# zhangzhousuper/Radish_PT

Measured on AMD Instinct MI355X. Metric: Mrays/s, higher is better.
Workload: dtype f32

## Files before the change

include/radish_hip.h:

```cpp
#ifndef RADISH_HIP_H
#define RADISH_HIP_H
#include <stdint.h>

#ifdef __cplusplus
extern "C" {
#endif

#define RDH_OK 0
#define RDH_ERR_ARGS (-1)
#define RDH_ERR_NO_SCENE (-2)
#define RDH_ERR_UNSUPPORTED (-3)
#define RDH_ERR_NO_DEVICE (-4)
#define RDH_ERR_STATE (-5)
#define RDH_ERR_COMM (-6)

typedef struct rdh_ctx rdh_ctx;

typedef struct rdh_texture { int32_t width, height; const float *data; } rdh_texture;

typedef struct rdh_scene_desc {
    const float *vertices;
    const float *normals;
    const float *texcoords;
    const float *boundingBoxes;
// ... 35 lines not shown
    uint64_t anyRays;
    uint64_t nodeVisits;
    uint64_t triTests;
    uint64_t closestHits;
} rdh_counters;

#define RDH_PT_MEGAKERNEL 0u
#define RDH_PT_WAVEFRONT 1u
#define RDH_PT_SORT_MATERIAL 2u
#define RDH_PT_COUNT 4u
#define RDH_PT_PERSISTENT 16u
#define RDH_PT_ONE_LANE_PER_PIXEL 64u
#define RDH_PT_MEGA_GBUFFER RDH_PT_ONE_LANE_PER_PIXEL
#define RDH_PT_WG_PER_RAY 256u
#define RDH_PT_NO_DEFER 128u
#define RDH_PT_PARTITION_GBUFFER 512u
#define RDH_PT_WF_SUBFRAMES 2048u
#define RDH_PT_RESTIR_FUSED 1024u
#define RDH_PT_WF_SMALL_LISTS 4096u
#define RDH_PT_PAIRS 32768u
#define RDH_PT_NO_PAIRS 16384u
#define RDH_PT_NO_PACKETS 8192u
#define RDH_PT_AUTO 65536u
#define RDH_PT_NO_SCHEDULE 32u
#define RDH_PT_PROFILE 8u

#define RDH_REUSE_TEMPORAL 1
#define RDH_REUSE_SPATIAL 2

typedef struct rdh_restir_params {
    int32_t reuseMask;
    int32_t risCount;
    int32_t numSpatial;
    int32_t temporalClamp;
    int32_t faithfulRIS;
} rdh_restir_params;

int rdh_create(rdh_ctx **out, int device);
void rdh_destroy(rdh_ctx *ctx);
const char *rdh_last_error(const rdh_ctx *ctx);
int rdh_set_stream(rdh_ctx *ctx, void *hipStream);
int rdh_synchronize(rdh_ctx *ctx);

int rdh_scene_upload(rdh_ctx *ctx, const rdh_scene_desc *desc);
typedef struct rdh_light_update {
    const void *lightSampler;
// ... 90 lines not shown
                                    const float *d_momentAccumIn, const float *d_colorIn, const rdh_gbuffer *gb, int first);
int rdh_denoise_estimate_variance(rdh_ctx *ctx, float *d_variance, const float *d_moment, int width, int height);
int rdh_denoise_filter_variance(rdh_ctx *ctx, float *d_varianceOut, const float *d_varianceIn, int width, int height);

int rdh_restir_read(rdh_ctx *ctx, int which, void *hostOut);
long long rdh_restir_read_scratch(rdh_ctx *ctx, int which, void *hostOut, long long maxBytes);

int rdh_trace_closest(rdh_ctx *ctx, const float *d_rays, int64_t n, rdh_hit *d_hits, uint32_t flags);
int rdh_trace_occluded(rdh_ctx *ctx, const float *d_segments, int64_t n, int32_t *d_occluded, uint32_t flags);

int rdh_dump_rays(rdh_ctx *ctx, int looper, int maxDepth, float *d_closest, int64_t capClosest, float *d_any, int64_t capAny,
                  int64_t *nClosest, int64_t *nAny);
int rdh_set_occupancy_share(rdh_ctx *ctx, int share);

int rdh_counters_reset(rdh_ctx *ctx);
int rdh_counters_read(rdh_ctx *ctx, rdh_counters *out);

int rdh_profile_reset(rdh_ctx *ctx);
int rdh_profile_read(rdh_ctx *ctx, double *totalMs, int64_t *launches);

int rdh_debug_persist_stamps(rdh_ctx *ctx, uint64_t *out5x4096);
int rdh_debug_persist_phases(rdh_ctx *ctx, uint64_t *out16);
int rdh_debug_wf_stamps(rdh_ctx *ctx, uint64_t *out, int64_t capacity, int32_t *stages, int32_t *waves);

int rdh_last_kernel_ms(rdh_ctx *ctx, float *ms);

#ifdef __cplusplus
}
#endif
#endif
```

radish_pt_amd/_build.py:

```python
import os
import subprocess
import sys

ROOT = os.path.dirname(os.path.dirname(os.path.abspath(__file__)))
CSRC = os.path.join(ROOT, "radish_pt_amd", "csrc")
HIPCC = os.environ.get("HIPCC", "/opt/rocm/bin/hipcc")

HOST_SOURCES = [os.path.join(CSRC, "host", "scene_build.cpp"), os.path.join(CSRC, "host", "scene_load.cpp")]
HIP_SOURCES = [os.path.join(CSRC, "radish_hip.hip")]
HIP_DEPS = [
    os.path.join(CSRC, "device", f)
    for f in ("rmath.h", "layouts.h", "traverse.h", "bsdf.h", "lights.h", "path_step.h", "kernels_pt.h", "kernels_restir.h", "kernels_wave.h", "kernels_persist.h", "kernels_walk.h", "wg_trace.h", "kernels_display.h", "kernels_denoise.h", "kernels_bvh.h", "kernels_refit.h", "kernels_lbvh.h", "kernels_lights.h", "kernels_pose.h", "kernels_materials.h", "kernels_textures.h", "display_math.h", "denoise_math.h", "reservoir.h")
] + [os.path.join(ROOT, "include", "radish_hip.h")]

HIP_FLAGS = [
    "--offload-arch=gfx950", "-O3", "-std=c++17", "-fPIC", "-shared", "-ffp-contract=off", "-fno-fast-math",
    "-fno-gpu-rdc", "-Wall", "-Wno-unused-function", "-Wno-unused-value", "-Wno-unused-result",
]


def _newer(target, deps):
    if not os.path.exists(target):
        return True
    t = os.path.getmtime(target)
    return any(os.path.exists(d) and os.path.getmtime(d) > t for d in deps)


def _run(cmd):
    print("[build]", " ".join(cmd), flush=True)
    subprocess.check_call(cmd)


def build_host(force=False):
    out = os.path.join(CSRC, "libradish_host.so")
    deps = HOST_SOURCES + [os.path.join(ROOT, "include", "radish_host.h")]
# ... 76 lines not shown
```

radish_pt_amd/api.py:

```python
import ctypes as C
import os

import numpy as np

from . import hostlib
from . import layouts as L

_HERE = os.path.dirname(os.path.abspath(__file__))
HIP_LIB_PATH = os.environ.get("RADISH_HIP_LIB") or os.path.join(_HERE, "csrc", "libradish_hip.so")

RDH_PT_MEGAKERNEL, RDH_PT_WAVEFRONT, RDH_PT_SORT_MATERIAL, RDH_PT_COUNT, RDH_PT_PROFILE = 0, 1, 2, 4, 8
RDH_PT_PERSISTENT = 16
RDH_PT_NO_SCHEDULE = 32
RDH_PT_ONE_LANE_PER_PIXEL = 64
RDH_PT_MEGA_GBUFFER = RDH_PT_ONE_LANE_PER_PIXEL
RDH_PT_NO_DEFER = 128
RDH_PT_WG_PER_RAY = 256
RDH_PT_PARTITION_GBUFFER = 512
RDH_PT_RESTIR_FUSED = 1024
RDH_PT_WF_SUBFRAMES = 2048
RDH_PT_WF_SMALL_LISTS = 4096
RDH_PT_NO_PAIRS = 16384
RDH_PT_NO_PACKETS = 8192
RDH_PT_PAIRS = 32768
RDH_PT_AUTO = 65536
RDH_BVH_SAH, RDH_BVH_LBVH = 0, 1
BVH_BUILDERS = {"sah": RDH_BVH_SAH, "lbvh": RDH_BVH_LBVH}
RDH_POSE_REFIT, RDH_POSE_SAH, RDH_POSE_LBVH = 0, 1, 2
RDH_POSE_REBUILD_LIGHTS = 1
POSE_TREES = {"refit": RDH_POSE_REFIT, "sah": RDH_POSE_SAH, "lbvh": RDH_POSE_LBVH}
OBJECT_RANGE_DTYPE = np.dtype([("firstPrim", "<i4"), ("numPrims", "<i4"), ("restFirstPrim", "<i4")])
SOBOL_SAMPLE_NUM = 10000

EXPORTS = [
    "rdh_create", "rdh_destroy", "rdh_last_error", "rdh_set_stream", "rdh_synchronize", "rdh_scene_upload",
    "rdh_scene_free", "rdh_set_camera", "rdh_set_partition", "rdh_tiles_per_rank", "rdh_untile", "rdh_path_trace", "rdh_path_trace_samples",
    "rdh_path_trace_direct", "rdh_gbuffer_render", "rdh_restir_init", "rdh_restir_free", "rdh_restir_direct",
    "rdh_restir_read", "rdh_restir_read_scratch", "rdh_copy_image_to_pbo", "rdh_denoise_eaw", "rdh_denoise_svgf", "rdh_denoise_modulate",
    "rdh_denoise_add", "rdh_denoise_temporal_accumulate", "rdh_denoise_estimate_variance", "rdh_denoise_filter_variance", "rdh_restir_exchange_pack", "rdh_restir_exchange_unpack", "rdh_trace_closest", "rdh_trace_occluded", "rdh_counters_reset", "rdh_counters_read",
    "rdh_last_kernel_ms", "rdh_profile_reset", "rdh_profile_read", "rdh_debug_persist_stamps", "rdh_debug_persist_phases", "rdh_debug_wf_stamps",
    "rdh_gbuffer_exchange_pack", "rdh_gbuffer_exchange_unpack", "rdh_comm_unique_id", "rdh_comm_init", "rdh_comm_destroy",
    "rdh_dump_rays", "rdh_set_occupancy_share", "rdh_allgather_tiles", "rdh_path_trace_gathered", "rdh_restir_exchange", "rdh_restir_direct_gathered", "rdh_gbuffer_exchange",
    "rdh_comm_init_all", "rdh_path_trace_gathered_all", "rdh_gbuffer_exchange_all", "rdh_restir_direct_gathered_all",
    "rdh_comm_set_overlap", "rdh_comm_join",
    "rdh_build_bvh_device", "rdh_scene_update_geometry", "rdh_debug_read_tree",
    "rdh_scene_refit_geometry", "rdh_scene_tree_cost",
    "rdh_build_bvh_device_ex", "rdh_scene_update_geometry_ex",
    "rdh_scene_track_motion",
    "rdh_build_alias_table_device", "rdh_scene_rebuild_lights", "rdh_debug_read_lights",
    "rdh_scene_set_objects", "rdh_scene_pose_objects", "rdh_debug_read_world",
    "rdh_scene_set_materials", "rdh_build_light_list_device",
    "rdh_scene_set_texture", "rdh_scene_env_power", "rdh_debug_read_textures",
    "rdh_scene_set_geometry", "rdh_debug_read_geometry",
]


class SceneDescC(C.Structure):
    _fields_ = [
        ("vertices", C.c_void_p), ("normals", C.c_void_p), ("texcoords", C.c_void_p), ("boundingBoxes", C.c_void_p),
        ("bvhNodes", C.c_void_p * 6), ("bvhSize", C.c_int32), ("numPrims", C.c_int32),
        ("materialIds", C.c_void_p), ("materials", C.c_void_p), ("numMaterials", C.c_int32),
        ("numLights", C.c_int32), ("lightPrimIds", C.c_void_p), ("lightUnitRadiance", C.c_void_p),
        ("sumLightPowerInv", C.c_float), ("lightSamplerLength", C.c_int32), ("lightSampler", C.c_void_p),
# ... 723 lines not shown

    def profile_reset(self):
        self.check(lib().rdh_profile_reset(self.h))

    def profile_read(self):
        ms, n = C.c_double(0), C.c_int64(0)
        self.check(lib().rdh_profile_read(self.h, C.byref(ms), C.byref(n)))
        return ms.value, n.value

    def debug_persist_stamps(self):
        out = np.zeros((5, 4096), dtype=np.uint64)
        self.check(lib().rdh_debug_persist_stamps(self.h, out.ctypes.data))
        return out

    def debug_wf_stamps(self):
        fn = lib().rdh_debug_wf_stamps
        fn.argtypes, fn.restype = [C.c_void_p, C.c_void_p, C.c_int64, C.POINTER(C.c_int32), C.POINTER(C.c_int32)], C.c_int32
        stages, waves = C.c_int32(0), C.c_int32(0)
        self.check(fn(self.h, None, 0, C.byref(stages), C.byref(waves)))
        out = np.zeros((stages.value, waves.value, 6), dtype=np.uint64)
        self.check(fn(self.h, out.ctypes.data, out.size, C.byref(stages), C.byref(waves)))
        return out

    def debug_persist_phases(self):
        out = np.zeros(16, dtype=np.uint64)
        self.check(lib().rdh_debug_persist_phases(self.h, out.ctypes.data))
        return out

    def last_kernel_ms(self):
        ms = C.c_float(0)
        self.check(lib().rdh_last_kernel_ms(self.h, C.byref(ms)))
        return ms.value


class ReservoirReuse:
    NONE, Temporal, Spatial, TemporalSpatial = 0, 1, 2, 3


class Settings:
    traceDepth = 0
    useReservoir = True
    reservoirReuse = ReservoirReuse.Temporal
    accumulate = False
    ptFlags = RDH_PT_PERSISTENT
    restirNumSpatial = 5
    restirRISCount = 32
# ... 262 lines not shown
```

radish_pt_amd/csrc/device/kernels_wave.h:

```cpp
#pragma once
#include "kernels_pt.h"
#include "wg_trace.h"

namespace rd {

constexpr int kWfLitCap = 8192;
constexpr int kWfLitShadow = 0x40000000;
constexpr int kMaxWaveDepth = 32;

struct alignas(128) WaveCounter {
    int v;
    int pad[31];
};
#ifndef RD_WF_TICKET_SHARDS
#define RD_WF_TICKET_SHARDS 8
#endif
constexpr int kTicketShards = RD_WF_TICKET_SHARDS;
struct WaveCounters {
    WaveCounter rayCount[kMaxWaveDepth + 2];
    WaveCounter shadowCount[kMaxWaveDepth + 2];
    WaveCounter litCount[kMaxWaveDepth + 2];
    WaveCounter traceHead[kMaxWaveDepth + 2];
    WaveCounter shadeHead[kMaxWaveDepth + 2][4];
    WaveCounter traceTicket[kMaxWaveDepth + 2][kTicketShards];
    WaveCounter shadeTicket[kMaxWaveDepth + 2][kTicketShards];
};

struct WaveWorkspace {
    float4 *ro[2];
    float4 *rd[2];
    float4 *thr[2];
    float4 *prevPos[2];
    float4 *accD;
    float4 *accI;
    float4 *nee[2];
    float4 *sht[2];
    uint2 *rng[2];
    int4 *hit;
    int *rayq[2];
    int *shadowq;
    int *litq[2];
    int litCap;
    int *treeOvf;
    int treeOvfDepth;
// ... 11 lines not shown
    const unsigned tag = __float_as_uint(n.w), kind = tag & 3u;
    if (kind == kWfNeeNone) return;
    float4 *acc = (kind == 0u ? w.accD : w.accI) + (tag >> 2);
    const float4 a = *acc;
    *acc = make_float4(a.x + n.x, a.y + n.y, a.z + n.z, 0.f);
}

RD_DEV Ray wfSlotRay(const WaveWorkspace &w, int set, int p, bool shadow, float &limit) {
    if (shadow) {
        const float4 x = w.prevPos[set][p], y = w.sht[set][p];
        return shadowRay(mk3(x.x, x.y, x.z), mk3(y.x, y.y, y.z), limit);
    }
    const float4 o = w.ro[set][p], d = w.rd[set][p];
    limit = 3.402823466e+38f;
    return Ray{mk3(o.x, o.y, o.z), mk3(d.x, d.y, d.z)};
}

struct WaveSlotPath {
    const WaveWorkspace &w;
    const int rs, p;
    const int wr, q;
    int home;
    const bool delta;
    RD_DEV v3 throughput() {
        const float4 t = w.thr[rs][p];
        home = __float_as_int(t.w);
        return mk3(t.x, t.y, t.z);
    }
    RD_DEV float samplePdf() const { return w.ro[rs][p].w; }
    RD_DEV bool sampleDelta() const { return delta; }
    RD_DEV v3 prevPos() const { const float4 c = w.prevPos[rs][p]; return mk3(c.x, c.y, c.z); }
    RD_DEV void setDirect(v3 v) { w.accD[home] = make_float4(v.x, v.y, v.z, 0.f); }
    RD_DEV void addIndirect(v3 v) { const float4 a = w.accI[home]; w.accI[home] = make_float4(a.x + v.x, a.y + v.y, a.z + v.z, 0.f); }
    RD_DEV Sampler rng(const DScene &s) const { const uint2 r = w.rng[rs][p]; return Sampler{s.sobol, r.x, (int)r.y}; }
    RD_DEV void setNee(v3 c, float nw) { w.nee[wr][q] = make_float4(c.x, c.y, c.z, wfNeeTag(home, nw < 0.f ? kWfNeeNone : (nw == 0.f ? 0u : 1u))); }
    RD_DEV void setPrevPos(v3 x) { w.prevPos[wr][q] = make_float4(x.x, x.y, x.z, 0.f); }
    RD_DEV void setRay(const Ray &ray, float pdf, bool deltaSample, v3 throughput, const Sampler &rng) {
        w.ro[wr][q] = make_float4(ray.o.x, ray.o.y, ray.o.z, pdf);
        w.rd[wr][q] = make_float4(ray.d.x, ray.d.y, ray.d.z, deltaSample ? 1.f : 0.f);
        w.thr[wr][q] = make_float4(throughput.x, throughput.y, throughput.z, __int_as_float(home));
        w.rng[wr][q] = make_uint2(rng.scramble, (unsigned)rng.ptr);
    }
};


RD_DEV void waveAppend(bool pred, int item, int *queue, int *count) {
    unsigned long long mask = __ballot(pred);
    if (mask == 0ull) return;
    int leader = __ffsll((long long)mask) - 1;
    int base = 0;
    if ((int)(threadIdx.x & 63u) == leader) base = atomicAdd(count, __popcll(mask));
    base = __shfl(base, leader, 64);
    if (pred) queue[base + __popcll(mask & laneMaskLt())] = item;
}

constexpr int kShadeChunks = 4;
constexpr int kShadePacket = 64 * kShadeChunks;
RD_DEV void waveAppendN(const bool (&pred)[kShadeChunks], const int (&item)[kShadeChunks], int *queue, int *count) {
// ... 380 lines not shown
        const unsigned long long doneM = __ballot(!alive && p >= 0);
        if (doneM != 0ull && __popcll(doneM) * 64 >= (__popcll(doneM) + __popcll(__ballot(alive))) * RD_WF_FINISH_MIN)
        if (!alive && p >= 0) {
            if (isShadow) {
                if (!occluded) wfAddNee(w, w.nee[set][p]);
            } else {
                bool hit = hitPrim != -1;
                if (hit) nHits++;
                w.hit[p] = make_int4(hitPrim, __float_as_int(hit ? hitBary.x : 0.f), __float_as_int(hit ? hitBary.y : 0.f),
                                     hit ? int(s.primClass[hitPrim]) : 0);
            }
            p = -1;
        }
    }
    RD_WF_STAMP(2);
    if (COUNT) flushCounters(s.counters, nClosest, nAny, nHits, ws);
}

constexpr int kSortChunks = 16;
constexpr int kSortPacket = 64 * kSortChunks;
#ifndef RD_WF_SHADE_WAVES
#define RD_WF_SHADE_WAVES 1
#endif
__global__ __launch_bounds__(256, RD_WF_SHADE_WAVES) void k_wf_shade(DScene s, WaveWorkspace w, int k, int maxDepth, int sorted) {
    __shared__ int sSorted[4][kSortPacket];
    WaveCounters *c = w.ctr;
    const int wg = workgroupTicket(c->shadeTicket[k]);
    const int lane = int(threadIdx.x & 63u);
    int *mySorted = sSorted[threadIdx.x >> 6];
    {
        const int q = 0;
        const int n = c->rayCount[k].v;
        const int *hitq = w.rayq[k & 1];
        int pendP[kShadeChunks], pendQ[kShadeChunks];
        bool pendShadow[kShadeChunks], pendRay[kShadeChunks];
#pragma unroll
        for (int j = 0; j < kShadeChunks; j++) {
            pendP[j] = pendQ[j] = -1;
            pendShadow[j] = pendRay[j] = false;
        }
        int packet = kShadePacket;
        if (sorted) {
            const int perWave = n / (2 * gridWaves());
            packet = ((perWave + kShadePacket - 1) / kShadePacket) * kShadePacket;
            packet = packet < kShadePacket ? kShadePacket : (packet > kSortPacket ? kSortPacket : packet);
        }
        int packetEnd = 0;
        for (int base = logicalWave(wg) * packet, sub = 0, fresh = 1;;) {
            if (sub == packet) {
// ... 26 lines not shown
                        if (in) mySorted[at + __popcll(m & laneMaskLt())] = pp[j];
                        at += __popcll(m);
                    }
                }
                __builtin_amdgcn_wave_barrier();
            }
            int item = base + sub + lane;
            const int subNow = sub;
            sub += 64;
            bool active = sorted ? (subNow + lane < packetEnd) : (item < n);
            bool emitShadow = false, emitRay = false, litShadow = false, litRay = false, rayFirst = false;
            int p = -1;
            const int q = base + subNow + lane;
            if (active) {
                p = sorted ? mySorted[subNow + lane] : hitq[item];
                if (p <= -2) p = -2 - p;
                active = p >= 0;
            }
            if (active) {
                const int4 h = w.hit[p];
                const float4 rdw = w.rd[k & 1][p];
                WaveSlotPath st{w, k & 1, p, (k + 1) & 1, q, p, rdw.w != 0.f};
                const PathStepResult r = pathStep(s, k, maxDepth, h.x, mk2(__int_as_float(h.y), __int_as_float(h.z)), mk3(rdw.x, rdw.y, rdw.z), st);
                if (r.shadow) {
                    w.sht[(k + 1) & 1][q] = make_float4(r.shadowTo.x, r.shadowTo.y, r.shadowTo.z, 0.f);
                    emitShadow = true;
                    const v3 dl = r.shadowTo - r.shadowFrom;
                    const float l2 = dot(dl, dl) * 1.21e-12f;
                    litShadow = dl.x * dl.x < l2 || dl.y * dl.y < l2 || dl.z * dl.z < l2;
                }
                if (r.extension) {
                    emitRay = true;
                    litRay = fabs_(r.ray.d.x) < 1.1e-6f || fabs_(r.ray.d.y) < 1.1e-6f || fabs_(r.ray.d.z) < 1.1e-6f;
                }
            }
            if (__ballot(litShadow || litRay) != 0ull) {
                int *lq = w.litq[(k + 1) & 1];
                int *lc = &c->litCount[k + 1].v;
                for (int kind = 0; kind < 2; kind++) {
                    const bool pred = kind == 0 ? litShadow : litRay;
                    const unsigned long long m = __ballot(pred);
                    if (m == 0ull) continue;
                    int at = 0;
                    if (lane == 0) at = atomicAdd(lc, __popcll(m));
                    at = __shfl(at, 0, 64) + __popcll(m & laneMaskLt());
                    if (pred && at < w.litCap) {
                        lq[at] = kind == 0 ? (q | kWfLitShadow) : q;
                        if (kind == 0) emitShadow = false;
                        else rayFirst = true;
                    }
                }
            }
            {
                const int j = ((sub >> 6) - 1) & (kShadeChunks - 1);
#pragma unroll
                for (int jj = 0; jj < kShadeChunks; jj++)
                    if (jj == j) {
                        pendP[jj] = q;
                        pendQ[jj] = rayFirst ? -2 - q : q;
                        pendShadow[jj] = emitShadow;
                        pendRay[jj] = emitRay;
                    }
            }
            if ((sub & (kShadePacket - 1)) == 0 || base + sub >= n) {
                waveAppendN(pendShadow, pendP, w.shadowq, &c->shadowCount[k].v);
                waveAppendN(pendRay, pendQ, w.rayq[(k + 1) & 1], &c->rayCount[k + 1].v);
#pragma unroll
                for (int jj = 0; jj < kShadeChunks; jj++) pendShadow[jj] = pendRay[jj] = false;
// ... 30 lines not shown
```

radish_pt_amd/csrc/radish_hip.hip:

```cpp
#include "radish_hip.h"

#include <hip/hip_runtime.h>
#include <dlfcn.h>

#include <algorithm>
#include <cfloat>
#include <climits>
#include <cmath>
#include <cstdarg>
#include <cstdio>
#include <cstring>
#include <mutex>
#include <string>
#include <type_traits>
#include <utility>
#include <vector>

#include "device/kernels_pt.h"
#include "device/kernels_restir.h"
#include "device/kernels_wave.h"
#include "device/kernels_persist.h"
#include "device/kernels_walk.h"
#include "device/kernels_display.h"
#include "device/kernels_denoise.h"
// ... 55 lines not shown
        epoch = 0;
    }
    void beginCall() {
        if (++epoch == 0) {
            std::fill(stamp.begin(), stamp.end(), 0u);
            epoch = 1;
        }
    }
    bool marked(size_t id) const { return stamp[id] == epoch; }
    bool mark(size_t id) {
        if (marked(id)) return false;
        stamp[id] = epoch;
        return true;
    }
};

struct SceneState {
    bool haveScene = false;
    DScene ds{};
    std::vector<void *> sceneAllocs;

    int *dLightPrims = nullptr;
    int numLights = 0;
    PairRec *updPairs = nullptr;
    bool treePending = false;

    bool planValid = false;
    bool treeRefit = false;

    TriRec *prevTris = nullptr;
    bool movedSinceRender = false;

    void *lightScratch = nullptr;
    bool lightsPending = false;

    std::vector<rdh_object_range> objects;
    StampSet posed;
    PoseArgs pose{};
    bool worldStale = false;

    std::vector<HostMaterial> hostMats;
    std::vector<int> matPrims;
    StampSet edited;
    int numTextures = 0;
    int lightCap = 0;
    int lightLenCap = 0;
// ... 49 lines not shown
    float4 *restirState = nullptr;
    long long restirPixels = 0;
    GrowBuf splitBuf{bufs};
    long long splitLastSlots = 0;
    bool restirFirstFrame = true;

    std::vector<hipEvent_t> profEvents;
    size_t profUsed = 0;

    void *comm = nullptr;
    hipStream_t commStream = nullptr;
    hipEvent_t evToComm = nullptr, evGbuf = nullptr, evImg = nullptr, evResv = nullptr;
    bool commOverlap = true;
    bool gbufPending = false;
    bool resvPending = false;
    GrowBuf commSend[2] = {GrowBuf{bufs}, GrowBuf{bufs}}, commRecv{bufs};

    WaveWorkspace wf[kWfParts] = {};
    hipStream_t wfStream = nullptr;
    hipEvent_t evWfJoin3 = nullptr;
    long long wfCapacity = 0;
    std::vector<void *> wfAllocs;
    hipEvent_t evWfFork = nullptr, evWfJoin = nullptr;
#ifdef RD_WF_STAMPS
    GrowBuf wfStamps{bufs};
    int wfStampStages = 0, wfStampWaves = 0;
#endif

    GrowBuf bvhScratch{bufs};
    GrowBuf lbvhScratch{bufs};
    GrowBuf updTree{bufs};
    GrowBuf dTreeHdr{bufs};
    GrowBuf hTreeHdr{bufs, true};
    hipEvent_t evTree = nullptr;
    StagePair aliasStage{bufs};
    hipEvent_t evUpdWait = nullptr;

    GrowBuf refitBuf{bufs};

    GrowBuf aliasScratch{bufs};
    GrowBuf hLightSums{bufs, true};
    hipEvent_t evLights = nullptr;

    StagePair poseStage{bufs};
    GrowBuf dPoseStage{bufs};

// ... 458 lines not shown
                return rc;
        }
        if ((rc = wfAlloc(c, &w.accD, n)) || (rc = wfAlloc(c, &w.accI, n)) ||
            (rc = wfAlloc(c, &w.hit, n)) || (rc = wfAlloc(c, &w.rayq[0], n)) || (rc = wfAlloc(c, &w.rayq[1], n)) ||
            (rc = wfAlloc(c, &w.shadowq, n)) || (rc = wfAlloc(c, &w.ctr, 1)) || (rc = wfAlloc(c, &w.litq[0], (size_t)kWfLitCap)) ||
            (rc = wfAlloc(c, &w.litq[1], (size_t)kWfLitCap)))
            return rc;
        w.litCap = 0;
    }
    if (!c->evWfFork) {
        int rc;
        if ((rc = newEvent(c, &c->evWfFork)) || (rc = newEvent(c, &c->evWfJoin))) return rc;
        HIP_TRY(c, hipStreamCreateWithFlags(&c->wfStream, hipStreamNonBlocking));
        if ((rc = newEvent(c, &c->evWfJoin3))) return rc;
    }
    c->wfCapacity = slots;
    return RDH_OK;
}

int wavefrontPathTrace(rdh_ctx *c, const PixelMap &pm, float *d_direct, float *d_indirect, int iter, int looper, int samples,
                       int maxDepth, uint32_t flags) {
    if (maxDepth > kMaxWaveDepth) return fail(c, RDH_ERR_ARGS, "maxDepth %d exceeds %d", maxDepth, kMaxWaveDepth);
    const bool count = (flags & RDH_PT_COUNT) != 0, sort = (flags & RDH_PT_SORT_MATERIAL) != 0;
    const bool tree = usePairs(c, flags);
    unsigned traceRes = 0, shadeRes = 0;
    int rq = RDH_OK;
    withBools([&](auto cnt, auto pr) { rq = residentGrid(c, k_wf_trace<cnt.value, pr.value>, 256, &traceRes); }, count, tree);
    if (rq || (rq = residentGrid(c, k_wf_shade, 256, &shadeRes))) return rq;
    if (tree && !count) {
        int cus = 0;
        if (int rc = cuCount(c, &cus)) return rc;
        traceRes = std::min(traceRes, (unsigned)cus * (unsigned)RD_WF_PAIR_MAX_WAVES);
    }
    const unsigned traceGrid = sharedGrid(c, std::min(traceRes, kPersistentGrid), kUnbounded);
    const unsigned shadeGrid = sharedGrid(c, std::min(shadeRes, kPersistentGrid), kUnbounded);
    static const int partsEnv = getenv("RADISH_WF_PARTS") ? atoi(getenv("RADISH_WF_PARTS")) : kWfPartsDefault;
    int parts = ((flags & RDH_PT_WF_SUBFRAMES) && pm.numBlocks >= 2048) ? (partsEnv >= 1 && partsEnv <= kWfParts ? partsEnv : kWfPartsDefault) : 1;
    const int ovfDepth = c->scene.ds.treeDepth + 1;
    const size_t ovfNeed = (size_t)traceGrid * 4 * 64 * (size_t)ovfDepth * 2;
    if (tree && parts > 1 && (size_t)parts * ovfNeed * sizeof(int) > kWfStripBudget) parts = 1;
    hipStream_t sts[kWfParts] = {c->stream, c->sideStream, c->wfStream};
    if (tree) {
        for (int h = 0; h < parts; h++) {
            if (int rc = grow(c, c->wfTreeOvf[h], ovfNeed, ovfNeed * sizeof(int), Busy::Device)) return rc;
            c->wf[h].treeOvf = c->wfTreeOvf[h].as<int>();
            c->wf[h].treeOvfDepth = ovfDepth;
        }
    }
#ifdef RD_WF_STAMPS
    {
        const size_t stamps = (size_t)(maxDepth + 1) * traceGrid * 4 * kWfStampKinds + (size_t)(maxDepth + 1);
        if (int rc = grow(c, c->wfStamps, stamps, stamps * sizeof(unsigned long long), Busy::Device)) return rc;
        HIP_TRY(c, hipMemsetAsync(c->wfStamps.p, 0, stamps * sizeof(unsigned long long), c->stream));
        for (int h = 0; h < kWfParts; h++) {
            c->wf[h].stamps = h == 0 ? c->wfStamps.as<unsigned long long>() : nullptr;
            c->wf[h].stampWaves = (int)(traceGrid * 4);
            c->wf[h].stampStages = maxDepth + 1;
        }
        c->wfStampStages = maxDepth + 1;
        c->wfStampWaves = (int)(traceGrid * 4);
    }
#endif
    const long pf = parts >= 2 ? profBegin(c, flags) : -1;
    if (parts >= 2) {
        HIP_TRY(c, hipEventRecord(c->evWfFork, c->stream));
        for (int h = 1; h < parts; h++) HIP_TRY(c, hipStreamWaitEvent(sts[h], c->evWfFork, 0));
    }
    int rc = RDH_OK;
    auto keep = [&](hipError_t e, const char *what) {
        if (e != hipSuccess && rc == RDH_OK) rc = fail(c, (int)e, "HIP error (%s:%d): %s: %s", __FILE__, __LINE__, what, hipGetErrorString(e));
    };
    for (int h = 0; h < parts; h++) {
        const unsigned waves = traceGrid * 4u;
        c->wf[h].litCap = (int)(waves * 64u < (unsigned)kWfLitCap ? waves * 64u : (unsigned)kWfLitCap);
        if (flags & RDH_PT_WF_SMALL_LISTS) c->wf[h].litCap = 4;
    }
    for (int h = 0; h < parts; h++) {
        hipStream_t st = sts[h];
        WaveWorkspace &w = c->wf[h];
        const unsigned nLocal = (unsigned)(pm.numBlocks - h + parts - 1) / (unsigned)parts;
        const unsigned gridBlk = (((nLocal * (unsigned)samples + 3u) / 4u + 7u) / 8u) * 8u;
        keep(hipMemsetAsync(w.ctr, 0, sizeof(WaveCounters), st), "hipMemsetAsync(wavefront counters)");
        hipLaunchKernelGGL(k_wf_raygen, dim3(gridBlk), dim3(256), 0, st, c->scene.ds, c->cam, pm, w, looper, samples, h, parts);
    }
    for (int k = 0; k <= maxDepth && rc == RDH_OK; k++) {
        for (int h = 0; h < parts; h++) {
            hipStream_t st = sts[h];
            WaveWorkspace &w = c->wf[h];
            long pe = (h == 0 && parts == 1) ? profBegin(c, flags) : -1;
            withBools([&](auto cnt, auto pr) {
                hipLaunchKernelGGL((k_wf_trace<cnt.value, pr.value>), dim3(traceGrid), dim3(256), 0, st, c->scene.ds, w, k);
            }, count, tree);
            profEnd(c, pe);
            hipLaunchKernelGGL(k_wf_shade, dim3(shadeGrid), dim3(256), 0, st, c->scene.ds, w, k, maxDepth, sort ? 1 : 0);
        }
        keep(hipGetLastError(), "wavefront stage launch");
    }
    for (int h = 0; h < parts && rc == RDH_OK; h++) {
        hipStream_t st = sts[h];
        const unsigned nLocal = (unsigned)(pm.numBlocks - h + parts - 1) / (unsigned)parts;
        const unsigned gridBlk = (((nLocal + 3u) / 4u + 7u) / 8u) * 8u;
        hipLaunchKernelGGL(k_wf_finish, dim3(gridBlk), dim3(256), 0, st, pm, c->wf[h], iter, samples, d_direct, d_indirect, h, parts);
    }
    keep(hipGetLastError(), "k_wf_finish");
    if (parts >= 2) {
        hipError_t e1 = hipEventRecord(c->evWfJoin, c->sideStream);
        hipError_t e2 = hipStreamWaitEvent(c->stream, c->evWfJoin, 0);
        hipError_t e3 = hipEventRecord(c->evWfJoin3, c->wfStream);
        hipError_t e4 = hipStreamWaitEvent(c->stream, c->evWfJoin3, 0);
        if (e1 != hipSuccess || e2 != hipSuccess || e3 != hipSuccess || e4 != hipSuccess) {
            hipStreamSynchronize(c->sideStream);
            hipStreamSynchronize(c->wfStream);
            keep(e1 != hipSuccess ? e1 : (e2 != hipSuccess ? e2 : (e3 != hipSuccess ? e3 : e4)), "wavefront join");
        }
    }
    profEnd(c, pf);
    return rc;
// ... 327 lines not shown
                               const_cast<LightPre *>(c->scene.ds.lightPre), (int)lights.size(), d->sumLightPowerInv);
            HIP_TRY(c, hipStreamSynchronize(c->stream));
        }
    }
    std::vector<AliasRec> alias(d->lightSamplerLength);
    if (d->lightSamplerLength) memcpy(alias.data(), d->lightSampler, sizeof(AliasRec) * alias.size());
    for (auto &e : alias)
        if (e.failId < 0 || e.failId >= d->lightSamplerLength) return fail(c, RDH_ERR_ARGS, "alias table failId out of range");
    if ((rc = uploadVec(c, alias, &c->scene.ds.lightAlias))) return rc;
    std::vector<uint32_t> sobol(d->sampleSequence, d->sampleSequence + 10000 * 200);
    if ((rc = uploadVec(c, sobol, &c->scene.ds.sobol))) return rc;

    c->scene.ds.counters = c->dCounters;
    c->scene.ds.bvhSize = S;
    c->scene.ds.numPrims = N;
    c->scene.ds.lightSamplerLength = d->lightSamplerLength;
    c->scene.ds.sumLightPowerInv = d->sumLightPowerInv;
    c->scene.lightCap = d->numLights;
    c->scene.lightLenCap = d->lightSamplerLength;
    c->scene.primCap = N;
    c->scene.hostMats.assign(hm, hm + d->numMaterials);
    c->scene.matPrims.assign((size_t)d->numMaterials, 0);
    for (int p = 0; p < N; p++) c->scene.matPrims[(size_t)d->materialIds[p]]++;
    c->scene.edited.reset((size_t)d->numMaterials);
    c->scene.numTextures = d->numTextures;
    c->scene.texInfo.assign(texInfo.begin(), texInfo.begin() + d->numTextures);
    c->scene.texFloats = texFloats;
    c->scene.haveScene = true;
    c->orderValid = false;
    return RDH_OK;
}

int rdh_set_camera(rdh_ctx *c, const void *camera196) {
    if (!c || !camera196) return RDH_ERR_ARGS;
    DCamera d = toDeviceCamera(camera196);
    if (d.resx <= 0 || d.resy <= 0) return fail(c, RDH_ERR_ARGS, "camera resolution %dx%d", d.resx, d.resy);
    if (d.resx != c->cam.resx || d.resy != c->cam.resy) c->orderValid = false;
    c->cam = d;
    c->haveCamera = true;
    return RDH_OK;
}

int rdh_set_partition(rdh_ctx *c, int rank, int world, int tileSize) {
    if (!c || world < 1 || rank < 0 || rank >= world || tileSize < 8 || (tileSize % 8) != 0)
        return fail(c, RDH_ERR_ARGS, "rdh_set_partition(rank=%d, world=%d, tile=%d)", rank, world, tileSize);
    if (rank != c->rank || world != c->world || tileSize != c->tile) c->orderValid = false;
// ... 1027 lines not shown
#ifdef RD_PERSIST_STAMPS
    HIP_TRY(c, hipStreamSynchronize(c->stream));
    HIP_TRY(c, hipMemcpy(out5x4096, c->dPersist->stamp, sizeof(unsigned long long) * 5 * 4096, hipMemcpyDeviceToHost));
    return RDH_OK;
#else
    return fail(c, RDH_ERR_UNSUPPORTED, "library built without RD_PERSIST_STAMPS");
#endif
}

int rdh_debug_wf_stamps(rdh_ctx *c, uint64_t *out, int64_t capacity, int32_t *stages, int32_t *waves) {
    if (!c || !stages || !waves || capacity < 0 || (capacity > 0 && !out)) return RDH_ERR_ARGS;
#ifdef RD_WF_STAMPS
    HIP_TRY(c, hipStreamSynchronize(c->stream));
    *stages = c->wfStampStages;
    *waves = c->wfStampWaves;
    const int64_t n = (int64_t)c->wfStampStages * c->wfStampWaves * kWfStampKinds;
    if (n > 0 && capacity >= n) HIP_TRY(c, hipMemcpy(out, c->wfStamps.p, sizeof(unsigned long long) * (size_t)n, hipMemcpyDeviceToHost));
    return RDH_OK;
#else
    return fail(c, RDH_ERR_UNSUPPORTED, "library built without RD_WF_STAMPS");
#endif
}

int rdh_copy_image_to_pbo(rdh_ctx *c, void *d_pbo, const void *d_image, int width, int height, int kind, int toneMapping,
                          float scale) {
    if (!c) return RDH_ERR_ARGS;
    if (!d_pbo || !d_image || width <= 0 || height <= 0 || kind < 0 || kind > 3 || toneMapping < 0 || toneMapping > 2)
        return fail(c, RDH_ERR_ARGS, "rdh_copy_image_to_pbo: bad arguments");
    HIP_TRY(c, hipSetDevice(c->device));
    if (int rj = joinComm(c)) return rj;
    long long total = (long long)width * height;
    hipLaunchKernelGGL(k_send_image_to_pbo, dim3((unsigned)((total + 255) / 256)), dim3(256), 0, c->stream,
                       static_cast<uint32_t *>(d_pbo), d_image, width, height, kind, toneMapping, scale);
    HIP_TRY(c, hipGetLastError());
    return RDH_OK;
}

extern "C++" {
namespace {
int denoiseGB(rdh_ctx *c, const rdh_gbuffer *gb, DenoiseGB &d, const char *what) {
    if (int rj = joinComm(c)) return rj;
    if (!gb || !gb->albedo || !gb->motion || gb->frameIdx < 0 || gb->frameIdx > 1 || gb->width <= 0 || gb->height <= 0)
        return fail(c, RDH_ERR_ARGS, "%s: bad G-buffer", what);
    for (int k = 0; k < 2; k++)
        if (!gb->normal[k] || !gb->depth[k] || !gb->primId[k]) return fail(c, RDH_ERR_ARGS, "%s: null G-buffer plane", what);
    const int f = gb->frameIdx;
// ... 1280 lines not shown
```

Baseline: 3063.

## Cull last-bounce rays missing emitter bounds and skip zero-contribution shadow rays

In the wavefront shade kernel, extension rays at the final bounce are no longer emitted when they cannot hit the bounding box of all emissive triangles (only with no environment map and a complete light list). Shadow rays whose NEE contribution is zero or absent are also no longer queued. A small per-frame kernel computes the padded emitter box. This cuts trace work on the last stage and on useless shadow rays, at the cost of an extra tiny launch, an extra atomic per wave for lit-shadow counting, and a new debug counter API.

```diff
diff --git a/include/radish_hip.h b/include/radish_hip.h
--- a/include/radish_hip.h
+++ b/include/radish_hip.h
@@ -81,6 +81,7 @@
 #define RDH_PT_NO_PAIRS 16384u
 #define RDH_PT_NO_PACKETS 8192u
 #define RDH_PT_AUTO 65536u
+#define RDH_PT_WALK_ALL 131072u
 #define RDH_PT_NO_SCHEDULE 32u
 #define RDH_PT_PROFILE 8u
 
@@ -217,6 +218,7 @@
 int rdh_debug_persist_stamps(rdh_ctx *ctx, uint64_t *out5x4096);
 int rdh_debug_persist_phases(rdh_ctx *ctx, uint64_t *out16);
 int rdh_debug_wf_stamps(rdh_ctx *ctx, uint64_t *out, int64_t capacity, int32_t *stages, int32_t *waves);
+int rdh_debug_wf_counts(rdh_ctx *ctx, int32_t *rays, int32_t *shadows, int32_t capacity, int32_t *stages);
 
 int rdh_last_kernel_ms(rdh_ctx *ctx, float *ms);
 
diff --git a/radish_pt_amd/_build.py b/radish_pt_amd/_build.py
--- a/radish_pt_amd/_build.py
+++ b/radish_pt_amd/_build.py
@@ -10,7 +10,7 @@
 HIP_SOURCES = [os.path.join(CSRC, "radish_hip.hip")]
 HIP_DEPS = [
     os.path.join(CSRC, "device", f)
-    for f in ("rmath.h", "layouts.h", "traverse.h", "bsdf.h", "lights.h", "path_step.h", "kernels_pt.h", "kernels_restir.h", "kernels_wave.h", "kernels_persist.h", "kernels_walk.h", "wg_trace.h", "kernels_display.h", "kernels_denoise.h", "kernels_bvh.h", "kernels_refit.h", "kernels_lbvh.h", "kernels_lights.h", "kernels_pose.h", "kernels_materials.h", "kernels_textures.h", "display_math.h", "denoise_math.h", "reservoir.h")
+    for f in ("rmath.h", "layouts.h", "traverse.h", "bsdf.h", "lights.h", "path_step.h", "kernels_pt.h", "kernels_restir.h", "kernels_wave.h", "ray_cull.h", "kernels_persist.h", "kernels_walk.h", "wg_trace.h", "kernels_display.h", "kernels_denoise.h", "kernels_bvh.h", "kernels_refit.h", "kernels_lbvh.h", "kernels_lights.h", "kernels_pose.h", "kernels_materials.h", "kernels_textures.h", "display_math.h", "denoise_math.h", "reservoir.h")
 ] + [os.path.join(ROOT, "include", "radish_hip.h")]
 
 HIP_FLAGS = [
diff --git a/radish_pt_amd/api.py b/radish_pt_amd/api.py
--- a/radish_pt_amd/api.py
+++ b/radish_pt_amd/api.py
@@ -24,6 +24,7 @@
 RDH_PT_NO_PACKETS = 8192
 RDH_PT_PAIRS = 32768
 RDH_PT_AUTO = 65536
+RDH_PT_WALK_ALL = 131072
 RDH_BVH_SAH, RDH_BVH_LBVH = 0, 1
 BVH_BUILDERS = {"sah": RDH_BVH_SAH, "lbvh": RDH_BVH_LBVH}
 RDH_POSE_REFIT, RDH_POSE_SAH, RDH_POSE_LBVH = 0, 1, 2
@@ -39,6 +40,7 @@
     "rdh_restir_read", "rdh_restir_read_scratch", "rdh_copy_image_to_pbo", "rdh_denoise_eaw", "rdh_denoise_svgf", "rdh_denoise_modulate",
     "rdh_denoise_add", "rdh_denoise_temporal_accumulate", "rdh_denoise_estimate_variance", "rdh_denoise_filter_variance", "rdh_restir_exchange_pack", "rdh_restir_exchange_unpack", "rdh_trace_closest", "rdh_trace_occluded", "rdh_counters_reset", "rdh_counters_read",
     "rdh_last_kernel_ms", "rdh_profile_reset", "rdh_profile_read", "rdh_debug_persist_stamps", "rdh_debug_persist_phases", "rdh_debug_wf_stamps",
+    "rdh_debug_wf_counts",
     "rdh_gbuffer_exchange_pack", "rdh_gbuffer_exchange_unpack", "rdh_comm_unique_id", "rdh_comm_init", "rdh_comm_destroy",
     "rdh_dump_rays", "rdh_set_occupancy_share", "rdh_allgather_tiles", "rdh_path_trace_gathered", "rdh_restir_exchange", "rdh_restir_direct_gathered", "rdh_gbuffer_exchange",
     "rdh_comm_init_all", "rdh_path_trace_gathered_all", "rdh_gbuffer_exchange_all", "rdh_restir_direct_gathered_all",
@@ -808,6 +810,16 @@
         self.check(fn(self.h, out.ctypes.data, out.size, C.byref(stages), C.byref(waves)))
         return out
 
+    def debug_wf_counts(self):
+        fn = lib().rdh_debug_wf_counts
+        fn.argtypes, fn.restype = [C.c_void_p, C.c_void_p, C.c_void_p, C.c_int32, C.POINTER(C.c_int32)], C.c_int32
+        stages = C.c_int32(0)
+        self.check(fn(self.h, None, None, 0, C.byref(stages)))
+        rays, shadows = np.zeros(stages.value, dtype=np.int32), np.zeros(stages.value, dtype=np.int32)
+        if stages.value:
+            self.check(fn(self.h, rays.ctypes.data, shadows.ctypes.data, stages.value, C.byref(stages)))
+        return rays, shadows
+
     def debug_persist_phases(self):
         out = np.zeros(16, dtype=np.uint64)
         self.check(lib().rdh_debug_persist_phases(self.h, out.ctypes.data))
diff --git a/radish_pt_amd/csrc/device/kernels_wave.h b/radish_pt_amd/csrc/device/kernels_wave.h
--- a/radish_pt_amd/csrc/device/kernels_wave.h
+++ b/radish_pt_amd/csrc/device/kernels_wave.h
@@ -1,6 +1,7 @@
 #pragma once
 #include "kernels_pt.h"
 #include "wg_trace.h"
+#include "ray_cull.h"
 
 namespace rd {
 
@@ -20,6 +21,7 @@
     WaveCounter rayCount[kMaxWaveDepth + 2];
     WaveCounter shadowCount[kMaxWaveDepth + 2];
     WaveCounter litCount[kMaxWaveDepth + 2];
+    WaveCounter litShadowCount[kMaxWaveDepth + 2];
     WaveCounter traceHead[kMaxWaveDepth + 2];
     WaveCounter shadeHead[kMaxWaveDepth + 2][4];
     WaveCounter traceTicket[kMaxWaveDepth + 2][kTicketShards];
@@ -77,6 +79,7 @@
     const int wr, q;
     int home;
     const bool delta;
+    bool nullNee = false;
     RD_DEV v3 throughput() {
         const float4 t = w.thr[rs][p];
         home = __float_as_int(t.w);
@@ -88,7 +91,10 @@
     RD_DEV void setDirect(v3 v) { w.accD[home] = make_float4(v.x, v.y, v.z, 0.f); }
     RD_DEV void addIndirect(v3 v) { const float4 a = w.accI[home]; w.accI[home] = make_float4(a.x + v.x, a.y + v.y, a.z + v.z, 0.f); }
     RD_DEV Sampler rng(const DScene &s) const { const uint2 r = w.rng[rs][p]; return Sampler{s.sobol, r.x, (int)r.y}; }
-    RD_DEV void setNee(v3 c, float nw) { w.nee[wr][q] = make_float4(c.x, c.y, c.z, wfNeeTag(home, nw < 0.f ? kWfNeeNone : (nw == 0.f ? 0u : 1u))); }
+    RD_DEV void setNee(v3 c, float nw) {
+        w.nee[wr][q] = make_float4(c.x, c.y, c.z, wfNeeTag(home, nw < 0.f ? kWfNeeNone : (nw == 0.f ? 0u : 1u)));
+        nullNee = nw < 0.f || (c.x == 0.f && c.y == 0.f && c.z == 0.f);
+    }
     RD_DEV void setPrevPos(v3 x) { w.prevPos[wr][q] = make_float4(x.x, x.y, x.z, 0.f); }
     RD_DEV void setRay(const Ray &ray, float pdf, bool deltaSample, v3 throughput, const Sampler &rng) {
         w.ro[wr][q] = make_float4(ray.o.x, ray.o.y, ray.o.z, pdf);
@@ -515,9 +521,23 @@
 #ifndef RD_WF_SHADE_WAVES
 #define RD_WF_SHADE_WAVES 1
 #endif
-__global__ __launch_bounds__(256, RD_WF_SHADE_WAVES) void k_wf_shade(DScene s, WaveWorkspace w, int k, int maxDepth, int sorted) {
+#ifndef RD_WF_CULL_LAST
+#define RD_WF_CULL_LAST 1
+#endif
+#ifndef RD_WF_SKIP_NULL_NEE
+#define RD_WF_SKIP_NULL_NEE 1
+#endif
+__global__ __launch_bounds__(256, RD_WF_SHADE_WAVES) void k_wf_shade(DScene s, WaveWorkspace w, int k, int maxDepth, int sorted,
+                                                                     const float4 *__restrict__ emitBox, int walkAll) {
     __shared__ int sSorted[4][kSortPacket];
     WaveCounters *c = w.ctr;
+    const bool cullLast = RD_WF_CULL_LAST && !walkAll && k + 1 == maxDepth && !hasEnvMap(s);
+    const bool skipNull = RD_WF_SKIP_NULL_NEE && !walkAll;
+    float4 boxLo = make_float4(0.f, 0.f, 0.f, 0.f), boxHi = boxLo;
+    if (cullLast) {
+        boxLo = emitBox[0];
+        boxHi = emitBox[1];
+    }
     const int wg = workgroupTicket(c->shadeTicket[k]);
     const int lane = int(threadIdx.x & 63u);
     int *mySorted = sSorted[threadIdx.x >> 6];
@@ -590,14 +610,14 @@
                 const float4 rdw = w.rd[k & 1][p];
                 WaveSlotPath st{w, k & 1, p, (k + 1) & 1, q, p, rdw.w != 0.f};
                 const PathStepResult r = pathStep(s, k, maxDepth, h.x, mk2(__int_as_float(h.y), __int_as_float(h.z)), mk3(rdw.x, rdw.y, rdw.z), st);
-                if (r.shadow) {
+                if (r.shadow && !(skipNull && st.nullNee)) {
                     w.sht[(k + 1) & 1][q] = make_float4(r.shadowTo.x, r.shadowTo.y, r.shadowTo.z, 0.f);
                     emitShadow = true;
                     const v3 dl = r.shadowTo - r.shadowFrom;
                     const float l2 = dot(dl, dl) * 1.21e-12f;
                     litShadow = dl.x * dl.x < l2 || dl.y * dl.y < l2 || dl.z * dl.z < l2;
                 }
-                if (r.extension) {
+                if (r.extension && !(cullLast && !mayReachEmitters(boxLo, boxHi, r.ray.o, r.ray.d))) {
                     emitRay = true;
                     litRay = fabs_(r.ray.d.x) < 1.1e-6f || fabs_(r.ray.d.y) < 1.1e-6f || fabs_(r.ray.d.z) < 1.1e-6f;
                 }
@@ -612,6 +632,10 @@
                     int at = 0;
                     if (lane == 0) at = atomicAdd(lc, __popcll(m));
                     at = __shfl(at, 0, 64) + __popcll(m & laneMaskLt());
+                    if (kind == 0) {
+                        const int listed = __popcll(__ballot(pred && at < w.litCap));
+                        if (lane == 0 && listed > 0) atomicAdd(&c->litShadowCount[k].v, listed);
+                    }
                     if (pred && at < w.litCap) {
                         lq[at] = kind == 0 ? (q | kWfLitShadow) : q;
                         if (kind == 0) emitShadow = false;
diff --git a/radish_pt_amd/csrc/device/ray_cull.h b/radish_pt_amd/csrc/device/ray_cull.h
--- /dev/null
+++ b/radish_pt_amd/csrc/device/ray_cull.h
@@ -0,0 +1,72 @@
+#pragma once
+#include "traverse.h"
+
+namespace rd {
+
+constexpr float kEmitPad = 0.0009765625f;
+
+RD_DEV bool mayReachEmitters(float4 lo, float4 hi, v3 o, v3 d) {
+    if (lo.w == 0.f) return false;
+    const float len2 = dot(d, d), l2 = len2 * 1.21e-12f;
+    if (!(d.x * d.x >= l2 && d.y * d.y >= l2 && d.z * d.z >= l2)) return true;
+    if (!(__builtin_fmaxf(__builtin_fmaxf(d.x * d.x, d.y * d.y), d.z * d.z) <= len2 * 0.999997f)) return true;
+    if (o.x >= lo.x && o.x <= hi.x && o.y >= lo.y && o.y <= hi.y && o.z >= lo.z && o.z <= hi.z) return true;
+    const float ix = 1.f / d.x, iy = 1.f / d.y, iz = 1.f / d.z;
+    const float ax = (lo.x - o.x) * ix, bx = (hi.x - o.x) * ix;
+    const float ay = (lo.y - o.y) * iy, by = (hi.y - o.y) * iy;
+    const float az = (lo.z - o.z) * iz, bz = (hi.z - o.z) * iz;
+    const float tNear = __builtin_fmaxf(__builtin_fmaxf(__builtin_fminf(ax, bx), __builtin_fminf(ay, by)), __builtin_fminf(az, bz));
+    const float tFar = __builtin_fminf(__builtin_fminf(__builtin_fmaxf(ax, bx), __builtin_fmaxf(ay, by)), __builtin_fmaxf(az, bz));
+    const bool miss = tFar < 0.f || tNear > tFar * 1.0000019073486328125f;
+    return !miss;
+}
+
+__global__ __launch_bounds__(256) void k_emitter_bounds(const TriRec *__restrict__ tris, const int *__restrict__ lightPrims, int numLights,
+                                                        const NodeRec *__restrict__ root, float4 *__restrict__ box) {
+    const float inf = __builtin_inff();
+    v3 lo = mk3(inf), hi = mk3(-inf);
+    for (int i = int(threadIdx.x); i < numLights; i += 256) {
+        const TriVerts t = loadTri(tris, lightPrims[i]);
+        lo.x = __builtin_fminf(lo.x, __builtin_fminf(t.a.x, __builtin_fminf(t.b.x, t.c.x)));
+        lo.y = __builtin_fminf(lo.y, __builtin_fminf(t.a.y, __builtin_fminf(t.b.y, t.c.y)));
+        lo.z = __builtin_fminf(lo.z, __builtin_fminf(t.a.z, __builtin_fminf(t.b.z, t.c.z)));
+        hi.x = __builtin_fmaxf(hi.x, __builtin_fmaxf(t.a.x, __builtin_fmaxf(t.b.x, t.c.x)));
+        hi.y = __builtin_fmaxf(hi.y, __builtin_fmaxf(t.a.y, __builtin_fmaxf(t.b.y, t.c.y)));
+        hi.z = __builtin_fmaxf(hi.z, __builtin_fmaxf(t.a.z, __builtin_fmaxf(t.b.z, t.c.z)));
+    }
+    for (int m = 32; m >= 1; m >>= 1) {
+        lo.x = __builtin_fminf(lo.x, __shfl_xor(lo.x, m, 64));
+        lo.y = __builtin_fminf(lo.y, __shfl_xor(lo.y, m, 64));
+        lo.z = __builtin_fminf(lo.z, __shfl_xor(lo.z, m, 64));
+        hi.x = __builtin_fmaxf(hi.x, __shfl_xor(hi.x, m, 64));
+        hi.y = __builtin_fmaxf(hi.y, __shfl_xor(hi.y, m, 64));
+        hi.z = __builtin_fmaxf(hi.z, __shfl_xor(hi.z, m, 64));
+    }
+    __shared__ float sLo[4][3], sHi[4][3];
+    if ((threadIdx.x & 63u) == 0u) {
+        const int wv = int(threadIdx.x >> 6);
+        sLo[wv][0] = lo.x, sLo[wv][1] = lo.y, sLo[wv][2] = lo.z;
+        sHi[wv][0] = hi.x, sHi[wv][1] = hi.y, sHi[wv][2] = hi.z;
+    }
+    __syncthreads();
+    if (threadIdx.x != 0) return;
+    for (int wv = 1; wv < 4; wv++) {
+        lo.x = __builtin_fminf(lo.x, sLo[wv][0]), lo.y = __builtin_fminf(lo.y, sLo[wv][1]), lo.z = __builtin_fminf(lo.z, sLo[wv][2]);
+        hi.x = __builtin_fmaxf(hi.x, sHi[wv][0]), hi.y = __builtin_fmaxf(hi.y, sHi[wv][1]), hi.z = __builtin_fmaxf(hi.z, sHi[wv][2]);
+    }
+    if (numLights <= 0) {
+        box[0] = make_float4(0.f, 0.f, 0.f, 0.f);
+        box[1] = make_float4(0.f, 0.f, 0.f, 0.f);
+        return;
+    }
+    float ext = __builtin_fmaxf(__builtin_fmaxf(hi.x - lo.x, hi.y - lo.y), hi.z - lo.z);
+    if (root) {
+        const float4 rl = root->lo_prim, rh = root->hi_next;
+        ext = __builtin_fmaxf(ext, __builtin_fmaxf(__builtin_fmaxf(rh.x - rl.x, rh.y - rl.y), rh.z - rl.z));
+    }
+    const float pad = ext * kEmitPad;
+    box[0] = make_float4(lo.x - pad, lo.y - pad, lo.z - pad, 1.f);
+    box[1] = make_float4(hi.x + pad, hi.y + pad, hi.z + pad, 0.f);
+}
+
+}
diff --git a/radish_pt_amd/csrc/radish_hip.hip b/radish_pt_amd/csrc/radish_hip.hip
--- a/radish_pt_amd/csrc/radish_hip.hip
+++ b/radish_pt_amd/csrc/radish_hip.hip
@@ -101,6 +101,8 @@
 
     int *dLightPrims = nullptr;
     int numLights = 0;
+    float4 *emitBox = nullptr;
+    bool lightListPartial = false;
     PairRec *updPairs = nullptr;
     bool treePending = false;
 
@@ -196,6 +198,7 @@
     long long wfCapacity = 0;
     std::vector<void *> wfAllocs;
     hipEvent_t evWfFork = nullptr, evWfJoin = nullptr;
+    int wfLastStages = 0, wfLastParts = 0;
 #ifdef RD_WF_STAMPS
     GrowBuf wfStamps{bufs};
     int wfStampStages = 0, wfStampWaves = 0;
@@ -700,6 +703,7 @@
                        int maxDepth, uint32_t flags) {
     if (maxDepth > kMaxWaveDepth) return fail(c, RDH_ERR_ARGS, "maxDepth %d exceeds %d", maxDepth, kMaxWaveDepth);
     const bool count = (flags & RDH_PT_COUNT) != 0, sort = (flags & RDH_PT_SORT_MATERIAL) != 0;
+    const bool walkAll = count || (flags & RDH_PT_WALK_ALL) != 0 || c->scene.lightListPartial;
     const bool tree = usePairs(c, flags);
     unsigned traceRes = 0, shadeRes = 0;
     int rq = RDH_OK;
@@ -739,6 +743,15 @@
         c->wfStampWaves = (int)(traceGrid * 4);
     }
 #endif
+    if (!c->scene.emitBox)
+        if (int rc = sceneAlloc(c, &c->scene.emitBox, 2 * sizeof(float4))) return rc;
+    if (RD_WF_CULL_LAST && !walkAll && maxDepth >= 1 && c->scene.ds.envTex < 0) {
+        hipLaunchKernelGGL(k_emitter_bounds, dim3(1), dim3(256), 0, c->stream, c->scene.ds.tris, (const int *)c->scene.dLightPrims,
+                           c->scene.numLights, c->scene.ds.bvhSize > 0 ? c->scene.ds.nodes[0] : nullptr, c->scene.emitBox);
+        HIP_TRY(c, hipGetLastError());
+    }
+    c->wfLastStages = maxDepth + 1;
+    c->wfLastParts = parts;
     const long pf = parts >= 2 ? profBegin(c, flags) : -1;
     if (parts >= 2) {
         HIP_TRY(c, hipEventRecord(c->evWfFork, c->stream));
@@ -770,7 +783,8 @@
                 hipLaunchKernelGGL((k_wf_trace<cnt.value, pr.value>), dim3(traceGrid), dim3(256), 0, st, c->scene.ds, w, k);
             }, count, tree);
             profEnd(c, pe);
-            hipLaunchKernelGGL(k_wf_shade, dim3(shadeGrid), dim3(256), 0, st, c->scene.ds, w, k, maxDepth, sort ? 1 : 0);
+            hipLaunchKernelGGL(k_wf_shade, dim3(shadeGrid), dim3(256), 0, st, c->scene.ds, w, k, maxDepth, sort ? 1 : 0,
+                               (const float4 *)c->scene.emitBox, walkAll ? 1 : 0);
         }
         keep(hipGetLastError(), "wavefront stage launch");
     }
@@ -1144,6 +1158,17 @@
     c->scene.hostMats.assign(hm, hm + d->numMaterials);
     c->scene.matPrims.assign((size_t)d->numMaterials, 0);
     for (int p = 0; p < N; p++) c->scene.matPrims[(size_t)d->materialIds[p]]++;
+    {
+        long long emissive = 0;
+        for (int m = 0; m < d->numMaterials; m++)
+            if (hm[m].type == kMaterialLight) emissive += c->scene.matPrims[(size_t)m];
+        bool complete = emissive == d->numLights;
+        for (int i = 0; complete && i < d->numLights; i++) {
+            const int p = d->lightPrimIds[i];
+            complete = hm[d->materialIds[p]].type == kMaterialLight && (i == 0 || p > d->lightPrimIds[i - 1]);
+        }
+        c->scene.lightListPartial = !complete;
+    }
     c->scene.edited.reset((size_t)d->numMaterials);
     c->scene.numTextures = d->numTextures;
     c->scene.texInfo.assign(texInfo.begin(), texInfo.begin() + d->numTextures);
@@ -2217,6 +2242,29 @@
 #endif
 }
 
+int rdh_debug_wf_counts(rdh_ctx *c, int32_t *rays, int32_t *shadows, int32_t capacity, int32_t *stages) {
+    if (!c || !stages || capacity < 0 || (capacity > 0 && (!rays || !shadows))) return RDH_ERR_ARGS;
+    HIP_TRY(c, hipSetDevice(c->device));
+    HIP_TRY(c, hipStreamSynchronize(c->stream));
+    *stages = c->wfLastStages;
+    if (c->wfLastStages <= 0 || capacity < c->wfLastStages) return RDH_OK;
+    std::fill(rays, rays + c->wfLastStages, 0);
+    std::fill(shadows, shadows + c->wfLastStages, 0);
+    std::vector<WaveCounter> host(3 * (size_t)c->wfLastStages);
+    const size_t bytes = sizeof(WaveCounter) * (size_t)c->wfLastStages;
+    for (int h = 0; h < c->wfLastParts; h++) {
+        const WaveCounters *d = c->wf[h].ctr;
+        HIP_TRY(c, hipMemcpy(host.data(), d->rayCount, bytes, hipMemcpyDeviceToHost));
+        HIP_TRY(c, hipMemcpy(host.data() + c->wfLastStages, d->shadowCount, bytes, hipMemcpyDeviceToHost));
+        HIP_TRY(c, hipMemcpy(host.data() + 2 * c->wfLastStages, d->litShadowCount, bytes, hipMemcpyDeviceToHost));
+        for (int k = 0; k < c->wfLastStages; k++) {
+            rays[k] += host[k].v;
+            shadows[k] += host[c->wfLastStages + k].v + host[2 * c->wfLastStages + k].v;
+        }
+    }
+    return RDH_OK;
+}
+
 int rdh_copy_image_to_pbo(rdh_ctx *c, void *d_pbo, const void *d_image, int width, int height, int kind, int toneMapping,
                           float scale) {
     if (!c) return RDH_ERR_ARGS;
```

Measured after the change: 3344 (median of 6 runs). 9.2% higher.
